# Grzetan/FPV-drone-RL-agent

Hardware: NVIDIA B200
Metric: env-steps/sec (physics+reward+obs), QuadX hover (higher is better)
Workload: dtype f32

## Files before the change

fpv-drone-rl-agent_b200/csrc/qx_kernels.cu:

```cuda
#include <cooperative_groups.h>
#include <cooperative_groups/reduce.h>
#include <cuda_bf16.h>
#include <cuda_runtime.h>

#include <atomic>
#include <cmath>
#include <cstddef>
#include <cstdio>
#include <cstdlib>
#include <cstring>
#include <type_traits>
#include <new>

#include "../../include/quadx_b200.h"
#include "qx_internal.h"
#include "qx_model.cuh"

namespace qx {

#ifndef QX_BLOCK
#define QX_BLOCK 128
#endif
#ifndef QX_MIN_BLOCKS
#define QX_MIN_BLOCKS 4
#endif
#ifndef QX_PAIR_UNROLL
#define QX_PAIR_UNROLL 1
#endif
constexpr int kBlock = QX_BLOCK;

struct Stats {
  double sum_ret;
  unsigned long long sum_len;
  unsigned long long n_done;
  unsigned long long n_nonfinite;
};

struct ResetQueue {
  unsigned int count;
  unsigned int ticket;
  unsigned int tasks_done, next_reset, exit_ticket, published;
  unsigned int pad[2];
  unsigned int idx[1];
};

struct StepArgs {
  float4* state;
  const float* actions;
  void* obs;
  float* reward;
  uint8_t* terminated;
  uint8_t* truncated;
  float* terminal_obs;
  const uint8_t* mask;
  Stats* stats;
  ResetQueue* queue;
  int64_t n;
  int64_t env_begin, env_count;
  int64_t obs_stride;
  int32_t k;
  int32_t obs_bf16;
  int32_t stream_stores;
  int32_t merged;
  uint32_t drainers;
  int32_t paired_reset;
};

template <int DIM>
__device__ __forceinline__ void write_obs(const float (&o)[DIM], void* base, int64_t row, int64_t stride, bool bf16, bool cs = false) {
  static_assert(DIM % 4 == 0, "obs rows are written as 16-byte / 8-byte vectors");
  if (bf16) {
    __nv_bfloat16* p = reinterpret_cast<__nv_bfloat16*>(base) + row * stride;
    if ((stride & 3) == 0) {
#pragma unroll
      for (int j = 0; j < DIM; j += 4) {
        __nv_bfloat162 a = __floats2bfloat162_rn(o[j], o[j + 1]), b = __floats2bfloat162_rn(o[j + 2], o[j + 3]);
        uint2 v;
        v.x = *reinterpret_cast<uint32_t*>(&a);
        v.y = *reinterpret_cast<uint32_t*>(&b);
        if (cs) __stcs(reinterpret_cast<uint2*>(p + j), v);
        else *reinterpret_cast<uint2*>(p + j) = v;
      }
    } else {
#pragma unroll
      for (int j = 0; j < DIM; ++j) p[j] = __float2bfloat16_rn(o[j]);
    }
  } else {
    float* p = reinterpret_cast<float*>(base) + row * stride;
    if ((stride & 3) == 0) {
#pragma unroll
      for (int j = 0; j < DIM; j += 4) {
        if (cs) __stcs(reinterpret_cast<float4*>(p + j), make_float4(o[j], o[j + 1], o[j + 2], o[j + 3]));
        else *reinterpret_cast<float4*>(p + j) = make_float4(o[j], o[j + 1], o[j + 2], o[j + 3]);
      }
    } else {
#pragma unroll
      for (int j = 0; j < DIM; ++j) p[j] = o[j];
    }
  }
}

enum { MODE_STEP_INLINE = 0, MODE_STEP_DEFER = 1, MODE_RESET_MASK = 2, MODE_RESET_QUEUE = 3 };

template <int MODE, int TASK, bool CASC, bool NC = true>
__device__ __forceinline__ void run_env(const DevConfig& c, const StepArgs& a, int64_t i);

constexpr int kResetQueueBlocks = 148 * 4;

__device__ __forceinline__ void publish_queue_length(ResetQueue* q) {
  __syncthreads();
  if (threadIdx.x == 0) {
    if (atomicAdd(&q->tasks_done, 1u) == gridDim.x - 1) {
      q->published = atomicAdd(&q->count, 0u);
      q->tasks_done = 0u;
    }
  }
}

template <int MODE, int TASK, bool CASC = false, bool REF = false>
__global__ void __launch_bounds__(kBlock, QX_MIN_BLOCKS) quadx_step_kernel(const __grid_constant__ DevConfig cparam, const __grid_constant__ StepArgs a) {
  if (MODE == MODE_STEP_INLINE) {
    asm volatile("griddepcontrol.wait;" ::: "memory");
    asm volatile("griddepcontrol.launch_dependents;");
  }
  DevConfig cref = cparam;
  if (REF) apply_ref_constants(cref);
  const DevConfig& c = REF ? cref : cparam;
  if (MODE == MODE_RESET_QUEUE) {
    const unsigned int cnt = *reinterpret_cast<volatile unsigned int*>(&a.queue->count);
    __syncthreads();
    if (threadIdx.x == 0) {
      __threadfence();
      if (atomicAdd(&a.queue->ticket, 1u) == gridDim.x - 1) { a.queue->count = 0u; a.queue->ticket = 0u; }
    }
    for (unsigned int t = blockIdx.x * kBlock + threadIdx.x; t < cnt; t += gridDim.x * kBlock)
      run_env<MODE, TASK, CASC>(c, a, (int64_t)a.queue->idx[t]);
  } else if (MODE == MODE_STEP_DEFER) {
    const int64_t i = a.env_begin + (int64_t)blockIdx.x * kBlock + threadIdx.x;
    if (i < a.env_begin + a.env_count) run_env<MODE, TASK, CASC>(c, a, i);
    publish_queue_length(a.queue);
  } else {
    const int64_t i = a.env_begin + (int64_t)blockIdx.x * kBlock + threadIdx.x;
    if (i >= a.env_begin + a.env_count) return;
    if (MODE == MODE_RESET_MASK && a.mask && !a.mask[i]) return;
    run_env<MODE, TASK, CASC>(c, a, i);
  }
}

__device__ __forceinline__ void respawn_cascade(Env& e, const DevConfig& c, float seul[3], float sp[4]) {
#pragma unroll
  for (int k = 0; k < 18; ++k) e.cp[k] = 0.f;
  quat_to_euler(e.sqx, e.sqy, e.sqz, e.sqw, seul[0], seul[1], seul[2]);
  sp[0] = sp[1] = sp[2] = sp[3] = 0.f;
  if (c.flight_mode == 2 || c.flight_mode == 3 || c.flight_mode == 4) sp[3] = e.spz;
  if (c.flight_mode == 7) { sp[0] = e.spx; sp[1] = e.spy; sp[2] = seul[2]; sp[3] = e.spz; }
}

template <int TASK> struct ObsDim { static constexpr int value = TASK == QX_TASK_HOVER ? QX_OBS_DIM_HOVER : QX_OBS_DIM_YAW; };
struct ObsAux { float er, ep, ey, cx, cy, area, ratio; bool vis; };

template <int TASK, bool RASTER_OK = true>
__device__ __forceinline__ void build_obs(Env& e, const DevConfig& c, const float act[4], const int phase, const bool live,
                                          float (&obs)[ObsDim<TASK>::value], ObsAux& x) {
  float er, ep, ey;
  if (phase == 0 && !live) {
    er = e.peul[0]; ep = e.peul[1]; ey = e.peul[2];
  } else {
    quat_to_euler(e.sqx, e.sqy, e.sqz, e.sqw, er, ep, ey);
  }
  if (phase == 1) { e.peul[0] = er; e.peul[1] = ep; e.peul[2] = ey; }
  const float two_pi = 6.28318530718f, pi = 3.14159265359f;
  float d0 = er - e.peul[0] + pi, d1 = ep - e.peul[1] + pi, d2 = ey - e.peul[2] + pi;
  d0 = d0 - two_pi * floorf(d0 * (1.f / two_pi)) - pi;
  d1 = d1 - two_pi * floorf(d1 * (1.f / two_pi)) - pi;
  d2 = d2 - two_pi * floorf(d2 * (1.f / two_pi)) - pi;
  bool vis;
  float cx, cy, area = 0.f, ratio = 0.f;
  if (TASK == QX_TASK_HOVER) {
    if (RASTER_OK && c.vision_mode == 1) vision_raster(e.px, e.py, e.pz, e.qx, e.qy, e.qz, e.qw, c.raster, vis, cx, cy, area, ratio);
    else vision(e, c, vis, cx, cy, area, ratio);
    obs[0] = d0 * c.inv_agent_dt; obs[1] = d1 * c.inv_agent_dt; obs[2] = d2 * c.inv_agent_dt;
    euler_to_quat(er, ep, ey, obs[3], obs[4], obs[5], obs[6]);
    obs[7] = cx; obs[8] = cy; obs[9] = e.pcx; obs[10] = e.pcy;
    obs[11] = area; obs[12] = e.parea; obs[13] = vis ? 1.f : 0.f; obs[14] = ratio; obs[15] = e.pratio;
    obs[16] = act[0]; obs[17] = act[1]; obs[18] = act[2]; obs[19] = act[3];
    e.pcx = cx; e.pcy = cy; e.parea = area; e.pratio = ratio;
  } else {
    vision_point(e, c, vis, cx, cy);
    const float k = c.inv_agent_dt * (1.f / 30.f);
    obs[0] = er * (1.f / pi); obs[1] = ep * (1.f / pi); obs[2] = ey * (1.f / pi);
    obs[3] = cx; obs[4] = cy;
    obs[5] = clampf(d0 * k, -1.f, 1.f); obs[6] = clampf(d1 * k, -1.f, 1.f); obs[7] = clampf(d2 * k, -1.f, 1.f);
    obs[8] = e.pa[0]; obs[9] = e.pa[1]; obs[10] = e.pa[2]; obs[11] = e.pa[3];
    e.pcx = cx; e.pcy = cy;
  }
  x.er = er; x.ep = ep; x.ey = ey; x.cx = cx; x.cy = cy; x.area = area; x.ratio = ratio; x.vis = vis;
}

template <int TASK, bool CASC>
__device__ __forceinline__ bool reward_and_flags(Env& e, const DevConfig& c, const StepArgs& a, const int64_t row, const float act[4],
                                                 const bool live, float (&obs)[ObsDim<TASK>::value], const ObsAux& x) {
  constexpr int OBS_DIM = ObsDim<TASK>::value;
  if (TASK == QX_TASK_YAW) {
    uint32_t fl = e.flags;
    if (e.step_count >= c.max_steps) fl |= F_TRUNC;
    if (e.spx * e.spx + e.spy * e.spy + e.spz * e.spz > c.dome2) fl |= F_OOB | F_TERM;
    const float reward = (x.vis ? 1.f - fabsf(x.cx) : -1.f) - 0.05f * fabsf(e.pa[3] - e.pa[2]);
    e.flags = fl;
    e.peul[0] = x.er; e.peul[1] = x.ep; e.peul[2] = x.ey;
    e.step_count += 1;
    e.rng_ctr += 1u;
    e.ep_ret += reward;
    a.reward[row] = reward;
    a.terminated[row] = (fl & F_TERM) ? 1 : 0;
    a.truncated[row] = (fl & F_TRUNC) ? 1 : 0;
    return c.auto_reset && (fl & (F_TERM | F_TRUNC));
  }
  float reward = -0.1f;
  uint32_t fl = e.flags;
  if (e.step_count > c.max_steps) fl |= F_TRUNC;
  if (live) {
    fl &= ~(F_LOWZ);
    if (e.spx * e.spx + e.spy * e.spy + e.spz * e.spz > c.dome2) fl |= F_OOB;
    if (e.spz < c.floor_thr) fl |= F_LOWZ;
  }
  bool bad = false;
  if (live && !(fabsf(e.px) + fabsf(e.py) + fabsf(e.pz) + fabsf(e.vx) + fabsf(e.vy) + fabsf(e.vz) + fabsf(e.wx) + fabsf(e.wy) + fabsf(e.wz) +
                fabsf(e.qw) < 3.0e38f)) {
    fl |= F_OOB;
    bad = true;
    atomicAdd(&a.stats->n_nonfinite, 1ull);
    e.px = e.py = 0.f; e.pz = c.floor_z; e.vx = e.vy = e.vz = 0.f; e.wx = e.wy = e.wz = 0.f; e.qx = e.qy = e.qz = 0.f; e.qw = 1.f;
#pragma unroll
    for (int m = 0; m < 4; ++m) e.thr[m] = 0.f;
#pragma unroll
    for (int ax = 0; ax < 3; ++ax) { e.pi[ax] = e.pe[ax] = e.swb[ax] = e.svb[ax] = 0.f; }
    if (CASC) {
#pragma unroll
      for (int k = 0; k < 18; ++k) e.cp[k] = 0.f;
      e.spx = e.spy = 0.f; e.spz = c.floor_z;
    }
  }
  if (fl & F_OOB) { reward = -100.f; fl |= F_TERM; }
  if (e.step_count > c.floor_grace && !c.render && (fl & F_LOWZ)) {
    reward = -100.f; fl |= F_TERM | F_ONFLOOR;
  }
  const float target_reward =
      x.vis ? -(fsqrt(x.cx * x.cx + x.cy * x.cy) + fabsf(x.area - c.target_area) + fabsf(x.ratio - c.target_ratio)) : -2.0f;
  reward -= 0.01f * e.swb[2] * e.swb[2];
  reward += target_reward - fsqrt(x.er * x.er + x.ep * x.ep);
  const float a0 = act[0] - e.pa[0], a1 = act[1] - e.pa[1], a2 = act[2] - e.pa[2], a3 = act[3] - e.pa[3];
  reward -= 0.2f * fsqrt(a0 * a0 + a1 * a1 + a2 * a2 + a3 * a3);
  reward += 1.0f;
  if (bad) {
    reward = -100.f;
#pragma unroll
    for (int j = 0; j < OBS_DIM; ++j) obs[j] = 0.f;
  }
  e.flags = fl;
  e.peul[0] = x.er; e.peul[1] = x.ep; e.peul[2] = x.ey;
  e.step_count += 1;
  e.pa[0] = act[0]; e.pa[1] = act[1]; e.pa[2] = act[2]; e.pa[3] = act[3];
  e.rng_ctr += 1u;
  e.ep_ret += reward;
  const bool term = fl & F_TERM, trunc = fl & F_TRUNC;
  if (a.stream_stores) {
    __stcs(a.reward + row, reward);
    __stcs(a.terminated + row, (uint8_t)(term ? 1 : 0));
    __stcs(a.truncated + row, (uint8_t)(trunc ? 1 : 0));
  } else {
    a.reward[row] = reward;
    a.terminated[row] = term ? 1 : 0;
    a.truncated[row] = trunc ? 1 : 0;
  }
  return c.auto_reset && (term || trunc);
}

template <bool DEFER, int OBS_DIM>
__device__ __forceinline__ void episode_end(const Env& e, const StepArgs& a, const int64_t i, const float (&obs)[OBS_DIM]) {
  namespace cg = cooperative_groups;
  const auto g = cg::coalesced_threads();
  const double sr = cg::reduce(g, (double)e.ep_ret, cg::plus<double>());
  const unsigned long long sl = cg::reduce(g, (unsigned long long)e.step_count, cg::plus<unsigned long long>());
  unsigned int base = 0;
  if (g.thread_rank() == 0) {
    atomicAdd(&a.stats->sum_ret, sr);
    atomicAdd(&a.stats->sum_len, sl);
// ... 199 lines not shown
  sp[3] = vfma(L::make(av0.w, av1.w), c.thrust_scale, c.thrust_bias);
  sp[3] = L::make(__saturatef(half_of<0>(sp[3])), __saturatef(half_of<1>(sp[3])));
  const uint32_t k0a = c.seed_lo ^ (c.env_lo + (uint32_t)i0), k0b = c.seed_lo ^ (c.env_lo + (uint32_t)i1);
  const uint32_t k1a = c.seed_hi ^ (c.env_hi + (uint32_t)(((uint64_t)c.env_lo + (uint64_t)i0) >> 32));
  const uint32_t k1b = c.seed_hi ^ (c.env_hi + (uint32_t)(((uint64_t)c.env_lo + (uint64_t)i1) >> 32));
  const int nsub = c.n_sub_step;
#pragma unroll 1
  for (int j = 0; j < nsub; j += 2) {
    V apwm[4];
    control_update<V>(p, c, sp, apwm);
    V nz[4] = {splat<V>(0.f), splat<V>(0.f), splat<V>(0.f), splat<V>(0.f)};
    uint4 ba = make_uint4(0u, 0u, 0u, 0u), bb = ba;
    if (c.noise) {
      ba = env_philox(make_uint4((uint32_t)j >> 1, STREAM_STEP, e0.rng_ctr, 0u), k0a, k1a);
      if (kLanes == 2) bb = env_philox(make_uint4((uint32_t)j >> 1, STREAM_STEP, e1.rng_ctr, 0u), k0b, k1b);
      if constexpr (kLanes == 2) normal4_scaled<V>(make_uint2(ba.x, bb.x), make_uint2(ba.y, bb.y), c.noise_k, nz);
      else normal4_scaled<V>(ba.x, ba.y, c.noise_k, nz);
    }
    physics_substep<V>(p, c, apwm, nz, false);
    if (c.noise) {
      if constexpr (kLanes == 2) normal4_scaled<V>(make_uint2(ba.z, bb.z), make_uint2(ba.w, bb.w), c.noise_k, nz);
      else normal4_scaled<V>(ba.z, ba.w, c.noise_k, nz);
    }
    physics_substep<V>(p, c, apwm, nz, j + 2 == nsub);
  }
  unpack_lane<0>(e0, p);
  if (kLanes == 2) unpack_lane<1>(e1, p);
}

#ifndef QX_SWP
#define QX_SWP 0
#endif
#ifndef QX_DIAG
#define QX_DIAG 0
#endif
#ifndef QX_RESET_SWP
#define QX_RESET_SWP 0
#endif
template <bool FLOOR = true, int SWP = QX_SWP>
QX_DI float substeps_s(const DevConfig& c, Env& e0, const f2 spxy, const float spz, const float thrust, const int nsub, const uint32_t stream, const int64_t i0) {
  CoreS p;
  pack_core_s(p, e0);
  float minz = __int_as_float(0x7f800000);
  const uint32_t k0 = c.seed_lo ^ (c.env_lo + (uint32_t)i0);
  const uint32_t k1 = c.seed_hi ^ (c.env_hi + (uint32_t)(((uint64_t)c.env_lo + (uint64_t)i0) >> 32));
  if constexpr (SWP == 0) {
#pragma unroll 1
  for (int j = 0; j < nsub; j += 2) {
    f2 apwm[2];
    control_update_s(p, c, spxy, spz, thrust, apwm);
    f2 nz[2] = {f2{0.f, 0.f}, f2{0.f, 0.f}};
    uint4 b = make_uint4(0u, 0u, 0u, 0u);
    if (c.noise) {
#if QX_DIAG == 2
      b = make_uint4(k0 + j, k1 ^ j, e0.rng_ctr * 0x9E3779B9u + j, k0 * 0x85EBCA6Bu + j);
#else
      b = env_philox(make_uint4((uint32_t)j >> 1, stream, e0.rng_ctr, 0u), k0, k1);
#endif
#if QX_DIAG == 1
      nz[0] = vmul(f2{__uint_as_float(0x3f800000u | (b.x >> 9)) - 1.5f, __uint_as_float(0x3f800000u | (b.x << 14 >> 9)) - 1.5f}, 0.02f);
      nz[1] = vmul(f2{__uint_as_float(0x3f800000u | (b.y >> 9)) - 1.5f, __uint_as_float(0x3f800000u | (b.y << 14 >> 9)) - 1.5f}, 0.02f);
#else
      normal4_scaled_s(b.x, b.y, c.noise_k, nz);
#endif
    }
    physics_substep_s<FLOOR>(p, c, apwm, nz, false, minz);
#if QX_DIAG == 1
    if (c.noise) {
      nz[0] = vmul(f2{__uint_as_float(0x3f800000u | (b.z >> 9)) - 1.5f, __uint_as_float(0x3f800000u | (b.z << 14 >> 9)) - 1.5f}, 0.02f);
      nz[1] = vmul(f2{__uint_as_float(0x3f800000u | (b.w >> 9)) - 1.5f, __uint_as_float(0x3f800000u | (b.w << 14 >> 9)) - 1.5f}, 0.02f);
    }
#else
    if (c.noise) normal4_scaled_s(b.z, b.w, c.noise_k, nz);
#endif
    physics_substep_s<FLOOR>(p, c, apwm, nz, j + 2 == nsub, minz);
  }
  } else if constexpr (SWP == 1) {
  uint4 b = make_uint4(0u, 0u, 0u, 0u);
  if (c.noise) b = env_philox(make_uint4(0u, stream, e0.rng_ctr, 0u), k0, k1);
#pragma unroll 1
  for (int j = 0; j < nsub; j += 2) {
    const uint4 bc = b;
    if (c.noise && j + 2 < nsub) b = env_philox(make_uint4(((uint32_t)j >> 1) + 1u, stream, e0.rng_ctr, 0u), k0, k1);
    f2 apwm[2];
    control_update_s(p, c, spxy, spz, thrust, apwm);
    f2 nz[2] = {f2{0.f, 0.f}, f2{0.f, 0.f}};
    if (c.noise) normal4_scaled_s(bc.x, bc.y, c.noise_k, nz);
    physics_substep_s<FLOOR>(p, c, apwm, nz, false, minz);
    if (c.noise) normal4_scaled_s(bc.z, bc.w, c.noise_k, nz);
    physics_substep_s<FLOOR>(p, c, apwm, nz, j + 2 == nsub, minz);
  }
  } else {
  f2 na[2] = {f2{0.f, 0.f}, f2{0.f, 0.f}}, nb[2] = {f2{0.f, 0.f}, f2{0.f, 0.f}};
  if (c.noise) {
    const uint4 b = env_philox(make_uint4(0u, stream, e0.rng_ctr, 0u), k0, k1);
    normal4_scaled_s(b.x, b.y, c.noise_k, na);
    normal4_scaled_s(b.z, b.w, c.noise_k, nb);
  }
#pragma unroll 1
  for (int j = 0; j < nsub; j += 2) {
    const f2 ca[2] = {na[0], na[1]}, cb[2] = {nb[0], nb[1]};
    if (c.noise && j + 2 < nsub) {
      const uint4 b = env_philox(make_uint4(((uint32_t)j >> 1) + 1u, stream, e0.rng_ctr, 0u), k0, k1);
      normal4_scaled_s(b.x, b.y, c.noise_k, na);
      normal4_scaled_s(b.z, b.w, c.noise_k, nb);
    }
    f2 apwm[2];
    control_update_s(p, c, spxy, spz, thrust, apwm);
    physics_substep_s<FLOOR>(p, c, apwm, ca, false, minz);
    physics_substep_s<FLOOR>(p, c, apwm, cb, j + 2 == nsub, minz);
  }
  }
  unpack_core_s(e0, p);
  return minz;
}
template <>
QX_DI void hot_substeps<S1>(const DevConfig& c, Env& e0, Env&, const float4 av0, const float4, const int64_t i0, const int64_t) {
  const f2 spxy = vmul(f2{av0.x, av0.y}, cpair(c.act_scale[0], c.act_scale[1]));
  const float spz = __fmul_rn(av0.z, c.act_scale[2]);
  const float thrust = __saturatef(fmaf(av0.w, c.thrust_scale, c.thrust_bias));
  substeps_s(c, e0, spxy, spz, thrust, c.n_sub_step, STREAM_STEP, i0);
}
#ifndef QX_SPEC_FLOOR
#define QX_SPEC_FLOOR 1
#endif
#ifndef QX_PREFETCH_TAIL
#define QX_PREFETCH_TAIL 1
#endif
QX_DI void hot_substeps_spec(const DevConfig& c, Env& e0, const StepArgs& a, const float4 av0, const int64_t i0) {
  const f2 spxy = vmul(f2{av0.x, av0.y}, cpair(c.act_scale[0], c.act_scale[1]));
  const float spz = __fmul_rn(av0.z, c.act_scale[2]);
  const float thrust = __saturatef(fmaf(av0.w, c.thrust_scale, c.thrust_bias));
  const float T = __fmul_rn((float)c.n_sub_step, c.h);
  const float reach = fmaf(fminf(e0.vz, 0.f), T, e0.pz) - __fmul_rn(__fmul_rn(c.g, T), T);
  const bool risky = e0.contact || !(reach > c.floor_z);
  const bool slow = __any_sync(__activemask(), risky);
  float minz = __int_as_float(0x7f800000);
  if (!slow) minz = substeps_s<false>(c, e0, spxy, spz, thrust, c.n_sub_step, STREAM_STEP, i0);
  const bool redo = minz < c.floor_z;
  if (slow || redo) {
    if (redo) load_env_loop(e0, a.state, a.n, i0);
    substeps_s<true>(c, e0, spxy, spz, thrust, c.n_sub_step, STREAM_STEP, i0);
  }
}

template <bool NC>
QX_DI void hot_reset_env(const DevConfig& c, const StepArgs& a, const int64_t i) {
  constexpr int OBS_DIM = QX_OBS_DIM_HOVER;
  Env e;
  load_env<NC>(e, a.state, a.n, i);
  const uint32_t k0 = c.seed_lo ^ (c.env_lo + (uint32_t)i);
  const uint32_t k1 = c.seed_hi ^ (c.env_hi + (uint32_t)(((uint64_t)c.env_lo + (uint64_t)i) >> 32));
  respawn(e, c, k0, k1);
  substeps_s<true, QX_RESET_SWP>(c, e, f2{0.f, 0.f}, 0.f, 0.f, c.n_sub_reset, STREAM_RESET, i);
  const float act[4] = {0.f, 0.f, 0.f, 0.f};
  float obs[OBS_DIM];
  ObsAux x;
  build_obs<QX_TASK_HOVER, false>(e, c, act, 1, true, obs, x);
  if (a.obs) write_obs(obs, a.obs, i, a.obs_stride, a.obs_bf16 != 0);
  store_env(e, a.state, a.n, i);
}
template <bool REF>
__device__ __noinline__ void hot_reset_requeue(const DevConfig& cparam, const StepArgs& a, const int64_t i) {
  DevConfig cref = cparam;
  if (REF) apply_ref_constants(cref);
  const DevConfig& c = REF ? cref : cparam;
  hot_reset_env<false>(c, a, i);
}

template <bool REF, class V>
QX_DI void hot_task(const DevConfig& c, const DevConfig& cparam, const StepArgs& a, const int64_t i0, const int64_t i1, const bool has1) {
  constexpr int kLanes = Lane<V>::N;
  Env e0, e1;
  const float4 av0 = __ldg(reinterpret_cast<const float4*>(a.actions) + i0);
  const float4 av1 = kLanes == 2 ? __ldg(reinterpret_cast<const float4*>(a.actions) + i1) : av0;
  load_env_loop(e0, a.state, a.n, i0);
  if (kLanes == 2) load_env_loop(e1, a.state, a.n, i1);
  if ((e0.flags | (kLanes == 2 ? e1.flags : 0u)) & (F_TERM | F_TRUNC)) {
    run_env_cold<REF>(cparam, a, i0);
    if (has1) run_env_cold<REF>(cparam, a, i1);
    return;
  }
#if QX_PREFETCH_TAIL
#pragma unroll
  for (int p = kLoopPlanes; p < 11; ++p) asm volatile("prefetch.global.L2 [%0];" ::"l"(a.state + (int64_t)p * a.n + i0));
#endif
  if constexpr (QX_SPEC_FLOOR && std::is_same<V, S1>::value) hot_substeps_spec(c, e0, a, av0, i0);
  else hot_substeps<V>(c, e0, e1, av0, av1, i0, i1);
  hot_epilogue<REF>(e0, c, a, i0, av0);
  if (has1) hot_epilogue<REF>(e1, c, a, i1, av1);
}

QX_DI unsigned int ld_acquire_u32(const unsigned int* p) {
  unsigned int v;
  asm volatile("ld.acquire.gpu.global.u32 %0, [%1];" : "=r"(v) : "l"(p) : "memory");
  return v;
}

template <bool REF, int SHAPE, class V, bool MERGED>
__global__ void __launch_bounds__(HotShape<SHAPE>::kBlock, HotShape<SHAPE>::kMinBlocks) quadx_step_hot_kernel(const __grid_constant__ DevConfig cparam,
                                                                                                                 const __grid_constant__ StepArgs a) {
  constexpr int kB = HotShape<SHAPE>::kBlock, kLanes = Lane<V>::N, kWarps = kB / 32, kTask = 32 * kLanes;
  if constexpr (!MERGED) {
    asm volatile("griddepcontrol.wait;" ::: "memory");
    asm volatile("griddepcontrol.launch_dependents;");
  }
  DevConfig cref = cparam;
  if (REF) apply_ref_constants(cref);
  const DevConfig& c = REF ? cref : cparam;
  const int64_t end = a.env_begin + a.env_count;
  const int64_t i0 = a.env_begin + ((int64_t)blockIdx.x * kWarps + (threadIdx.x >> 5)) * kTask + (threadIdx.x & 31u);
  if (i0 < end) {
    const bool has1 = kLanes == 2 && i0 + 32 < end;
    hot_task<REF, V>(c, cparam, a, i0, has1 ? i0 + 32 : i0, has1);
  }
  if constexpr (!MERGED) {
    if (a.queue) publish_queue_length(a.queue);
  }
  if constexpr (MERGED) {
    ResetQueue* const q = a.queue;
    __shared__ unsigned int s_ticket;
    __syncthreads();
    if (threadIdx.x == 0) s_ticket = atomicAdd(&q->tasks_done, 1u);
    __syncthreads();
    if (s_ticket + a.drainers < gridDim.x) return;
    if (threadIdx.x == 0) {
      unsigned int ns = 64u;
      while (ld_acquire_u32(&q->tasks_done) < gridDim.x) { __nanosleep(ns); if (ns < 512u) ns += ns; }
    }
    __syncthreads();
    const unsigned int cnt = ld_acquire_u32(&q->count);
#pragma unroll 1
    while (cnt != 0u) {
      unsigned int r = 0u;
      if ((threadIdx.x & 31u) == 0u) r = atomicAdd(&q->next_reset, 32u);
      r = __shfl_sync(0xffffffffu, r, 0);
      if (r >= cnt) break;
      if (r + (threadIdx.x & 31u) < cnt) {
        const int64_t ie = (int64_t)__ldcg(&q->idx[r + (threadIdx.x & 31u)]);
        if (a.paired_reset) hot_reset_requeue<REF>(cparam, a, ie);
        else run_env_requeue<REF>(cparam, a, ie);
      }
      __syncwarp();
    }
    __syncthreads();
    if (threadIdx.x == 0) {
      const unsigned int n_drain = a.drainers < gridDim.x ? a.drainers : gridDim.x;
      if (atomicAdd(&q->exit_ticket, 1u) == n_drain - 1u) {
        q->published = cnt; q->count = 0u; q->tasks_done = 0u; q->next_reset = 0u; q->exit_ticket = 0u;
      }
    }
  }
}

template <bool REF>
__global__ void __launch_bounds__(128, 4) quadx_reset_hot_kernel(const __grid_constant__ DevConfig cparam, const __grid_constant__ StepArgs a) {
  DevConfig cref = cparam;
  if (REF) apply_ref_constants(cref);
  const DevConfig& c = REF ? cref : cparam;
  asm volatile("griddepcontrol.wait;" ::: "memory");
  asm volatile("griddepcontrol.launch_dependents;");
  const unsigned int cnt = *reinterpret_cast<volatile unsigned int*>(&a.queue->count);
  __syncthreads();
  if (threadIdx.x == 0) {
    __threadfence();
    if (atomicAdd(&a.queue->ticket, 1u) == gridDim.x - 1) { a.queue->count = 0u; a.queue->ticket = 0u; }
  }
  for (unsigned int t = blockIdx.x * 128 + threadIdx.x; t < cnt; t += gridDim.x * 128) hot_reset_env<true>(c, a, (int64_t)a.queue->idx[t]);
}

__global__ void clock_probe_kernel(unsigned long long* out) {
  unsigned long long ns;
  asm volatile("mov.u64 %0, %%globaltimer;" : "=l"(ns));
  out[0] = (unsigned long long)clock64();
  out[1] = ns;
}

}

struct QxHandle {
  QxConfig cfg;
  qx::DevConfig dev;
  int64_t n;
  int device;
  int planes;
  bool ref_constants;
  bool hot_ok;
  int hot_mode;
  int paired_reset;
  int hot_lanes;
  int hot_shape;
  int stream_stores;
  int merged;
  int sm_count;
  int pdl;
  int host_chunks;
  int host_one_d2h;
  int hot_grid;
  float4* state;
  qx::Stats* stats;
  qx::ResetQueue* queue;
  float* raster;
  cudaStream_t stream, h2d_stream, d2h_stream, d2h2_stream;
  cudaEvent_t ev_h2d[16], ev_k[16], ev_d2h;
  float* h_act; float* d_act;
  float* h_obs; float* d_obs;
  float* h_rew; float* d_rew;
  uint8_t* h_flags; uint8_t* d_flags;
  float* h_tobs; float* d_tobs;
  bool staging;
};

static thread_local char g_err[512] = "";
static std::atomic<int64_t> g_launches{0};

int qx_fail(int code, const char* fmt, const char* detail) {
  snprintf(g_err, sizeof(g_err), fmt, detail);
  return code;
}
static int fail(int code, const char* fmt, const char* detail = "") { return qx_fail(code, fmt, detail); }
#define QX_CUDA(call)                                                             \
  do {                                                                            \
    cudaError_t _e = (call);                                                      \
    if (_e != cudaSuccess) return fail(QX_ECUDA, #call ": %s", cudaGetErrorString(_e)); \
  } while (0)

extern "C" const char* qx_last_error(void) { return g_err; }
extern "C" int32_t qx_version(void) { return QX_VERSION; }
extern "C" int64_t qx_launch_count(void) { return g_launches.load(); }
extern "C" int64_t qx_sizeof_config(void) { return (int64_t)sizeof(QxConfig); }

extern "C" int qx_default_config(int32_t task, QxConfig* c) {
  if (!c || (task != QX_TASK_HOVER && task != QX_TASK_YAW)) return fail(QX_EINVAL, "qx_default_config: bad arguments");
  memset(c, 0, sizeof(*c));
  c->task = task;
  c->mass = 0.1f;
  c->inertia[0] = 3e-5f; c->inertia[1] = 3e-5f; c->inertia[2] = 5e-5f;
  const float mx[4] = {0.028f, -0.028f, 0.028f, -0.028f}, my[4] = {-0.028f, 0.028f, 0.028f, -0.028f};
  const float ts[4] = {-1.f, -1.f, 1.f, 1.f};
  const float map[16] = {-1, -1, -1, 1, 1, 1, -1, 1, 1, -1, 1, 1, -1, 1, 1, 1};
  memcpy(c->motor_x, mx, sizeof(mx)); memcpy(c->motor_y, my, sizeof(my));
  memcpy(c->torque_sign, ts, sizeof(ts)); memcpy(c->motor_map, map, sizeof(map));
  c->total_thrust = 4.0f; c->thrust_coef = 3.16e-10f; c->torque_coef = 7.94e-12f; c->noise_ratio = 0.02f; c->tau = 0.01f;
  c->drag_coef_xyz = 1.5f; c->drag_area_xyz = 3.0e-4f; c->drag_coef_pqr = 1.0e-4f; c->air_density = 1.225f;
  const float kp[3] = {2.0e-2f, 2.0e-2f, 4.0e-2f}, ki[3] = {2.5e-7f, 2.5e-7f, 1.35e-4f}, kd[3] = {5.0e-5f, 5.0e-5f, 0.f};
  for (int a = 0; a < 3; ++a) { c->rate_kp[a] = kp[a]; c->rate_ki[a] = ki[a]; c->rate_kd[a] = kd[a]; c->rate_lim[a] = 1.0f; }
  c->pwm_idle = 0.05f; c->physics_hz = 240.f; c->control_hz = 120.f; c->gravity = 9.81f;
  c->state_stale = 1; c->gyro = 1; c->max_coord_vel = 100.f; c->floor_z = 0.01f;
  c->cam_tilt_up_deg = 25.f; c->cam_fov_deg = 90.f; c->cam_res = 128.f; c->cam_near = 0.1f; c->vis_margin_px = 0.5f;
  const float panel[12] = {4.98f, -1, 5, 4.98f, 1, 5, 4.98f, 1, 7, 4.98f, -1, 7};
  memcpy(c->panel, panel, sizeof(panel));
  for (int k = 0; k < 4; ++k) { c->panel_back[3 * k] = panel[3 * k] + 0.04f; c->panel_back[3 * k + 1] = panel[3 * k + 1]; c->panel_back[3 * k + 2] = panel[3 * k + 2]; }
  c->vision_mode = 0;
  c->aviary_steps_per_step = task == QX_TASK_HOVER ? 6 : 1;
  c->max_steps = 400; c->floor_grace_steps = 30; c->reset_idle_steps = task == QX_TASK_HOVER ? 10 : 0;
  c->agent_dt = 0.025f; c->flight_dome_size = 3.0f; c->floor_threshold = 0.1f;
  c->target_area = 0.013f; c->target_ratio = 1.53f;
  c->action_scale[0] = 30.f; c->action_scale[1] = 30.f; c->action_scale[2] = -30.f;
  c->spawn_yaw_noise = task == QX_TASK_YAW ? 3.14159265f : 0.f;
  if (task == QX_TASK_YAW) {
    c->cam_tilt_up_deg = -20.f;
    c->panel[0] = 2.f; c->panel[1] = 0.f; c->panel[2] = 1.f;
    c->agent_dt = 1.0f / 120.f;
  }
  c->render = 0; c->auto_reset = 1; c->noise = 1;
  c->flight_mode = 0; c->thrust_scale = 0.5f; c->thrust_bias = 0.5f;
  const float att[12] = {1, 1, 1, 0, 0, 0, 0, 0, 0, 2, 2, 2};
  const float vel[8] = {0.4f, 0.4f, 0.15f, 0.15f, 0.25f, 0.25f, 0.3f, 0.3f};
  const float pos[8] = {0.5f, 0.5f, 0, 0, 0, 0, 1, 1};
  const float zp[4] = {0.8f, 0, 0, 1.5f}, zv[4] = {1.5f, 0.3f, 0.05f, 1.0f};
  memcpy(c->att_pid, att, sizeof(att)); memcpy(c->vel_pid, vel, sizeof(vel)); memcpy(c->pos_pid, pos, sizeof(pos));
  memcpy(c->zpos_pid, zp, sizeof(zp)); memcpy(c->zvel_pid, zv, sizeof(zv));
  return QX_OK;
}

static int derive(const QxConfig& s, uint64_t seed, uint64_t env_id0, qx::DevConfig* d) {
  memset(d, 0, sizeof(*d));
  if (s.task != QX_TASK_HOVER && s.task != QX_TASK_YAW) return fail(QX_EINVAL, "qx_create: unknown task");
  if (!(s.physics_hz > 0) || !(s.control_hz > 0) || s.control_hz > s.physics_hz) return fail(QX_EINVAL, "qx_create: bad rates");
  if (s.flight_mode < -1 || s.flight_mode > 7) return fail(QX_EINVAL, "qx_create: flight_mode outside PyFlyt's -1..7");
  if (s.flight_mode != 0 && s.task != QX_TASK_HOVER) return fail(QX_EINVAL, "qx_create: flight modes other than 0 apply to the hover task");
  if (s.vision_mode != 0 && s.vision_mode != 1) return fail(QX_EINVAL, "qx_create: vision_mode is 0 (analytic) or 1 (raster)");
  const int per = (int)(s.physics_hz / s.control_hz);
  d->task = s.task;
  d->ctrl_every = per;
  d->n_sub_step = s.aviary_steps_per_step * per;
  d->n_sub_reset = s.reset_idle_steps * per;
  d->max_steps = s.max_steps; d->floor_grace = s.floor_grace_steps; d->render = s.render; d->auto_reset = s.auto_reset;
  d->noise = (s.noise && s.noise_ratio != 0.f) ? 1 : 0;
  d->state_stale = s.state_stale; d->gyro = s.gyro;
  d->obs_dim = s.task == QX_TASK_HOVER ? QX_OBS_DIM_HOVER : QX_OBS_DIM_YAW;
  d->act_dim = s.task == QX_TASK_HOVER ? QX_ACT_DIM_HOVER : QX_ACT_DIM_YAW;
  const double h = 1.0 / s.physics_hz, T = 1.0 / s.control_hz;
  d->h = (float)h; d->lag_alpha = (float)(h / s.tau); d->one_m_alpha = (float)(1.0 - h / s.tau); d->noise_ratio = s.noise_ratio;
  d->noise_k = (float)(-2.0 * M_LN2 * (double)s.noise_ratio * (double)s.noise_ratio);
  d->thrust_k = (float)(s.total_thrust / 4.0); d->pwm_idle = s.pwm_idle;
  const double max_rpm2 = s.total_thrust / (4.0 * s.thrust_coef);
  for (int m = 0; m < 4; ++m) {
    d->torque_k[m] = (float)(s.torque_sign[m] * s.torque_coef * max_rpm2);
    d->mx[m] = s.motor_x[m]; d->my[m] = s.motor_y[m];
  }
  memcpy(d->map, s.motor_map, sizeof(d->map));
  d->drag_c = (float)(0.5 * s.air_density * s.drag_coef_xyz * s.drag_area_xyz); d->drag_pqr = s.drag_coef_pqr;
  for (int a = 0; a < 3; ++a) {
    d->kp[a] = s.rate_kp[a]; d->kiT[a] = (float)(s.rate_ki[a] * T); d->kd_T[a] = (float)(s.rate_kd[a] / T); d->lim[a] = s.rate_lim[a];
    d->I[a] = s.inertia[a]; d->invI[a] = (float)(1.0 / s.inertia[a]);
    d->cam_off[a] = s.cam_offset[a]; d->act_scale[a] = s.action_scale[a];
    d->start_pos[a] = s.start_pos[a]; d->start_rpy[a] = s.start_rpy[a];
  }
  d->inv_mass = (float)(1.0 / s.mass); d->g = s.gravity; d->vmax = s.max_coord_vel; d->floor_z = s.floor_z;
  for (int a = 0; a < 3; ++a) {
    d->hI[a] = (float)(h / s.inertia[a]);
    d->gk[a] = s.gyro ? (float)(-(h / s.inertia[a]) * ((double)s.inertia[(a + 2) % 3] - (double)s.inertia[(a + 1) % 3])) : 0.f;
  }
  d->hm = (float)(h / s.mass); d->hg = (float)(h * s.gravity); d->hh = (float)(0.5 * h); d->hh2 = (float)(0.25 * h * h);
  d->kq1 = (float)(-0.5 * h / 6.0); d->kq2 = (float)(0.5 * h / 120.0);
  d->ndrag_c = -(float)(0.5 * s.air_density * s.drag_coef_xyz * s.drag_area_xyz); d->ndrag_pqr = -s.drag_coef_pqr;
  const double tilt = s.cam_tilt_up_deg * M_PI / 180.0;
  d->cam_sd = (float)sin(tilt); d->cam_cd = (float)cos(tilt);
  d->inv_tan = (float)(1.0 / tan(0.5 * s.cam_fov_deg * M_PI / 180.0));
// ... 115 lines not shown
  return QX_OK;
}

struct DeviceGuard {
  int prev = 0;
  explicit DeviceGuard(int d) { cudaGetDevice(&prev); cudaSetDevice(d); }
  ~DeviceGuard() { cudaSetDevice(prev); }
};

extern "C" int qx_nonfinite_count(QxHandle* h, int64_t* count) {
  if (!h || !count) return fail(QX_EINVAL, "qx_nonfinite_count: bad arguments");
  DeviceGuard g(h->device);
  qx::Stats s;
  QX_CUDA(cudaMemcpy(&s, h->stats, sizeof(s), cudaMemcpyDeviceToHost));
  *count = (int64_t)s.n_nonfinite;
  return QX_OK;
}

extern "C" int64_t qx_num_envs(const QxHandle* h) { return h ? h->n : 0; }
extern "C" int32_t qx_obs_dim(const QxHandle* h) { return h ? h->dev.obs_dim : 0; }
extern "C" int32_t qx_act_dim(const QxHandle* h) { return h ? h->dev.act_dim : 0; }
extern "C" void* qx_state_ptr(QxHandle* h) { return h ? h->state : nullptr; }
extern "C" int32_t qx_state_words(const QxHandle* h) { return h ? 4 * h->planes : 0; }
static bool matches_ref_constants(const qx::DevConfig& d) {
  qx::DevConfig lit = d;
  qx::apply_ref_constants(lit);
  return QX_HAVE_REF_CONSTANTS && d.task == QX_TASK_HOVER && d.flight_mode == 0 && memcmp(&lit, &d, sizeof(lit)) == 0;
}
extern "C" int32_t qx_uses_reference_constants(const QxHandle* h) { return h && h->ref_constants ? 1 : 0; }
extern "C" int32_t qx_config_matches_reference_constants(const QxConfig* cfg) {
  qx::DevConfig d;
  if (!cfg || derive(*cfg, 0, 0, &d) != QX_OK) return -1;
  return matches_ref_constants(d) ? 1 : 0;
}
extern "C" int64_t qx_debug_dev_config(const QxConfig* cfg, uint64_t seed, uint64_t env_id0, void* out, int64_t cap) {
  qx::DevConfig d;
  if (!cfg || derive(*cfg, seed, env_id0, &d) != QX_OK) return -1;
  if (out && cap >= (int64_t)sizeof(d)) memcpy(out, &d, sizeof(d));
  return (int64_t)sizeof(d);
}

template <int TASK, bool CASC, bool REF>
static void launch_task(QxHandle* h, int mode, const qx::StepArgs& a, cudaStream_t s) {
  const unsigned grid = (unsigned)((a.env_count + qx::kBlock - 1) / qx::kBlock);
  switch (mode) {
    case qx::MODE_STEP_INLINE:
      if (h->pdl) {
        cudaLaunchConfig_t lc{};
        lc.gridDim = dim3(grid); lc.blockDim = dim3(qx::kBlock); lc.dynamicSmemBytes = 0; lc.stream = s;
        cudaLaunchAttribute at{};
        at.id = cudaLaunchAttributeProgrammaticStreamSerialization;
        at.val.programmaticStreamSerializationAllowed = 1;
        lc.attrs = &at; lc.numAttrs = 1;
        cudaLaunchKernelEx(&lc, qx::quadx_step_kernel<qx::MODE_STEP_INLINE, TASK, CASC, REF>, h->dev, a);
      } else {
        qx::quadx_step_kernel<qx::MODE_STEP_INLINE, TASK, CASC, REF><<<grid, qx::kBlock, 0, s>>>(h->dev, a);
      }
      break;
    case qx::MODE_STEP_DEFER: qx::quadx_step_kernel<qx::MODE_STEP_DEFER, TASK, CASC, REF><<<grid, qx::kBlock, 0, s>>>(h->dev, a); break;
    case qx::MODE_RESET_MASK: qx::quadx_step_kernel<qx::MODE_RESET_MASK, TASK, CASC, REF><<<grid, qx::kBlock, 0, s>>>(h->dev, a); break;
    default: {
      const unsigned g = grid < (unsigned)qx::kResetQueueBlocks ? grid : (unsigned)qx::kResetQueueBlocks;
      qx::quadx_step_kernel<qx::MODE_RESET_QUEUE, TASK, CASC, REF><<<g, qx::kBlock, 0, s>>>(h->dev, a);
      break;
    }
  }
}

static bool stream_is_capturing(cudaStream_t s) {
  cudaStreamCaptureStatus st = cudaStreamCaptureStatusNone;
  return cudaStreamIsCapturing(s, &st) == cudaSuccess && st != cudaStreamCaptureStatusNone;
}

template <bool REF, int SHAPE, class V>
static cudaError_t launch_hot_kernel(QxHandle* h, const qx::StepArgs& a, cudaStream_t s) {
  constexpr int B = qx::HotShape<SHAPE>::kBlock, per = 32 * qx::Lane<V>::N, warps = B / 32;
  const int64_t n_tasks = (a.env_count + per - 1) / per;
  unsigned grid = (unsigned)((n_tasks + warps - 1) / warps);
  if (a.merged) {
    if (h->hot_grid == 0) {
      int per_sm = 0;
      cudaError_t e = cudaOccupancyMaxActiveBlocksPerMultiprocessor(&per_sm, qx::quadx_step_hot_kernel<REF, SHAPE, V, true>, B, 0);
      if (e != cudaSuccess) return e;
      h->hot_grid = h->sm_count * (per_sm > 0 ? per_sm : 1);
    }
    qx::StepArgs am = a;
    am.drainers = (uint32_t)h->hot_grid;
    qx::quadx_step_hot_kernel<REF, SHAPE, V, true><<<grid, B, 0, s>>>(h->dev, am);
    return cudaSuccess;
  }
  if (h->pdl && !stream_is_capturing(s)) {
    cudaLaunchConfig_t lc{};
    lc.gridDim = dim3(grid); lc.blockDim = dim3(B); lc.dynamicSmemBytes = 0; lc.stream = s;
    cudaLaunchAttribute at{};
    at.id = cudaLaunchAttributeProgrammaticStreamSerialization;
    at.val.programmaticStreamSerializationAllowed = 1;
    lc.attrs = &at; lc.numAttrs = 1;
    return cudaLaunchKernelEx(&lc, qx::quadx_step_hot_kernel<REF, SHAPE, V, false>, h->dev, a);
  }
  qx::quadx_step_hot_kernel<REF, SHAPE, V, false><<<grid, B, 0, s>>>(h->dev, a);
  return cudaSuccess;
}
template <int SHAPE, class V>
static cudaError_t launch_hot_one(QxHandle* h, const qx::StepArgs& a, cudaStream_t s) {
  return h->ref_constants ? launch_hot_kernel<true, SHAPE, V>(h, a, s) : launch_hot_kernel<false, SHAPE, V>(h, a, s);
}
template <class V>
static cudaError_t launch_hot_shape(QxHandle* h, const qx::StepArgs& a, cudaStream_t s) {
  switch (h->hot_shape) {
    case 3: return launch_hot_one<3, V>(h, a, s);
    case 4: return launch_hot_one<4, V>(h, a, s);
    case 5: return launch_hot_one<5, V>(h, a, s);
    default: return launch_hot_one<0, V>(h, a, s);
  }
}
static bool use_merged(const QxHandle* h);
static int launch_hot(QxHandle* h, int mode, qx::StepArgs a, cudaStream_t s) {
  if (a.env_count == 0) { a.env_begin = 0; a.env_count = h->n; }
  a.stream_stores = h->stream_stores;
  a.merged = (mode == qx::MODE_STEP_DEFER && use_merged(h)) ? h->merged : 0;
  a.paired_reset = h->paired_reset;
  if (a.merged) a.queue = h->queue;
  cudaError_t e;
#ifdef QX_EXTRA_SHAPES
  if (h->hot_lanes == 4 && h->hot_shape >= 6) {
    switch (h->hot_shape) {
      case 6: e = launch_hot_one<6, qx::S1>(h, a, s); break;
      case 7: e = launch_hot_one<7, qx::S1>(h, a, s); break;
      case 8: e = launch_hot_one<8, qx::S1>(h, a, s); break;
      default: e = launch_hot_one<9, qx::S1>(h, a, s); break;
    }
  } else
#endif
  if (h->hot_lanes == 2) e = launch_hot_shape<qx::P2<true>>(h, a, s);
  else if (h->hot_lanes == 4) e = launch_hot_shape<qx::S1>(h, a, s);
  else e = launch_hot_shape<float>(h, a, s);
  QX_CUDA(e);
  ++g_launches;
  QX_CUDA(cudaGetLastError());
  return QX_OK;
}
constexpr int64_t kHotMinEnvs = 32768;
static bool use_hot(const QxHandle* h) {
  if (!h->hot_ok || h->hot_mode == 0) return false;
  return h->hot_mode == 1 || h->n >= kHotMinEnvs;
}
static bool use_merged(const QxHandle* h) { return use_hot(h) && h->cfg.auto_reset && h->merged; }

static int launch(QxHandle* h, int mode, qx::StepArgs a, cudaStream_t s) {
  if (a.env_count == 0) { a.env_begin = 0; a.env_count = h->n; }
  if (use_hot(h) && (mode == qx::MODE_STEP_DEFER || (mode == qx::MODE_STEP_INLINE && a.k == 1 && !h->cfg.auto_reset)))
    return launch_hot(h, mode, a, s);
  if (mode == qx::MODE_RESET_QUEUE && use_hot(h) && h->paired_reset) {
    const unsigned blocks = (unsigned)((a.env_count + 127) / 128);
    const unsigned g = blocks < (unsigned)qx::kResetQueueBlocks ? blocks : (unsigned)qx::kResetQueueBlocks;
    if (h->pdl && !stream_is_capturing(s)) {
      cudaLaunchConfig_t lc{};
      lc.gridDim = dim3(g); lc.blockDim = dim3(128); lc.dynamicSmemBytes = 0; lc.stream = s;
      cudaLaunchAttribute at{};
      at.id = cudaLaunchAttributeProgrammaticStreamSerialization;
      at.val.programmaticStreamSerializationAllowed = 1;
      lc.attrs = &at; lc.numAttrs = 1;
      QX_CUDA(h->ref_constants ? cudaLaunchKernelEx(&lc, qx::quadx_reset_hot_kernel<true>, h->dev, a)
                               : cudaLaunchKernelEx(&lc, qx::quadx_reset_hot_kernel<false>, h->dev, a));
    } else if (h->ref_constants) qx::quadx_reset_hot_kernel<true><<<g, 128, 0, s>>>(h->dev, a);
    else qx::quadx_reset_hot_kernel<false><<<g, 128, 0, s>>>(h->dev, a);
    ++g_launches;
    QX_CUDA(cudaGetLastError());
    return QX_OK;
  }
  if (h->dev.task == QX_TASK_YAW) launch_task<QX_TASK_YAW, false, false>(h, mode, a, s);
  else if (h->dev.flight_mode != 0) launch_task<QX_TASK_HOVER, true, false>(h, mode, a, s);
  else if (h->ref_constants) launch_task<QX_TASK_HOVER, false, true>(h, mode, a, s);
  else launch_task<QX_TASK_HOVER, false, false>(h, mode, a, s);
  ++g_launches;
  QX_CUDA(cudaGetLastError());
  return QX_OK;
}

extern "C" int qx_reset(QxHandle* h, const uint8_t* mask_dev, void* obs_dev, int32_t obs_dtype, int64_t obs_stride, void* stream) {
  if (!h) return fail(QX_EINVAL, "qx_reset: null handle");
  if (obs_dev && obs_stride < h->dev.obs_dim) return fail(QX_EINVAL, "qx_reset: obs_stride < obs_dim");
  qx::StepArgs a{};
  a.state = h->state; a.mask = mask_dev; a.obs = obs_dev; a.obs_stride = obs_stride; a.obs_bf16 = obs_dtype == QX_OBS_BF16;
  a.stats = h->stats; a.n = h->n; a.k = 1;
  return launch(h, qx::MODE_RESET_MASK, a, (cudaStream_t)stream);
}

extern "C" int qx_step_k(QxHandle* h, int32_t k, const float* actions_dev, float* obs_dev, float* reward_dev,
                         uint8_t* terminated_dev, uint8_t* truncated_dev, void* stream) {
  if (!h || k <= 0 || !actions_dev || !reward_dev || !terminated_dev || !truncated_dev)
    return fail(QX_EINVAL, "qx_step_k: bad arguments");
  qx::StepArgs a{};
  a.state = h->state; a.actions = actions_dev; a.obs = obs_dev; a.obs_stride = h->dev.obs_dim; a.reward = reward_dev;
  a.terminated = terminated_dev; a.truncated = truncated_dev; a.stats = h->stats; a.n = h->n; a.k = k;
  return launch(h, qx::MODE_STEP_INLINE, a, (cudaStream_t)stream);
}

extern "C" int qx_step_begin(QxHandle* h, const float* actions_dev, void* obs_dev, int32_t obs_dtype, int64_t obs_stride,
                             float* reward_dev, uint8_t* terminated_dev, uint8_t* truncated_dev, float* terminal_obs_dev, void* stream) {
  if (!h || !actions_dev || !reward_dev || !terminated_dev || !truncated_dev) return fail(QX_EINVAL, "qx_step: bad arguments");
  if (obs_dev && obs_stride < h->dev.obs_dim) return fail(QX_EINVAL, "qx_step: obs_stride < obs_dim");
  qx::StepArgs a{};
  a.state = h->state; a.actions = actions_dev; a.obs = obs_dev; a.obs_stride = obs_stride; a.obs_bf16 = obs_dtype == QX_OBS_BF16;
  a.reward = reward_dev; a.terminated = terminated_dev; a.truncated = truncated_dev; a.terminal_obs = terminal_obs_dev;
  a.stats = h->stats; a.n = h->n; a.k = 1;
  if (!h->cfg.auto_reset) return launch(h, qx::MODE_STEP_INLINE, a, (cudaStream_t)stream);
  a.queue = h->queue;
  return launch(h, qx::MODE_STEP_DEFER, a, (cudaStream_t)stream);
}

extern "C" int qx_step_end(QxHandle* h, void* obs_dev, int32_t obs_dtype, int64_t obs_stride, void* stream) {
  if (!h) return fail(QX_EINVAL, "qx_step_end: null handle");
  if (!h->cfg.auto_reset) return QX_OK;
  if (obs_dev && obs_stride < h->dev.obs_dim) return fail(QX_EINVAL, "qx_step_end: obs_stride < obs_dim");
  if (use_merged(h)) return QX_OK;
  qx::StepArgs a{};
  a.state = h->state; a.obs = obs_dev; a.obs_stride = obs_stride; a.obs_bf16 = obs_dtype == QX_OBS_BF16;
  a.stats = h->stats; a.queue = h->queue; a.n = h->n; a.k = 1;
  return launch(h, qx::MODE_RESET_QUEUE, a, (cudaStream_t)stream);
}

constexpr int64_t kInlineResetMaxEnvs = 16384;
extern "C" int qx_step(QxHandle* h, const float* actions_dev, void* obs_dev, int32_t obs_dtype, int64_t obs_stride,
                       float* reward_dev, uint8_t* terminated_dev, uint8_t* truncated_dev, float* terminal_obs_dev, void* stream) {
  if (h && h->cfg.auto_reset && h->n <= kInlineResetMaxEnvs && !(h->hot_mode == 1 && h->hot_ok)) {
    if (!actions_dev || !reward_dev || !terminated_dev || !truncated_dev) return fail(QX_EINVAL, "qx_step: bad arguments");
    if (obs_dev && obs_stride < h->dev.obs_dim) return fail(QX_EINVAL, "qx_step: obs_stride < obs_dim");
    qx::StepArgs a{};
    a.state = h->state; a.actions = actions_dev; a.obs = obs_dev; a.obs_stride = obs_stride; a.obs_bf16 = obs_dtype == QX_OBS_BF16;
    a.reward = reward_dev; a.terminated = terminated_dev; a.truncated = truncated_dev; a.terminal_obs = terminal_obs_dev;
    a.stats = h->stats; a.n = h->n; a.k = 1;
    return launch(h, qx::MODE_STEP_INLINE, a, (cudaStream_t)stream);
  }
  int rc = qx_step_begin(h, actions_dev, obs_dev, obs_dtype, obs_stride, reward_dev, terminated_dev, truncated_dev, terminal_obs_dev, stream);
  if (rc) return rc;
  return qx_step_end(h, obs_dev, obs_dtype, obs_stride, stream);
}

extern "C" int qx_debug_clock_probe(unsigned long long* out_dev, void* stream) {
  if (!out_dev) return fail(QX_EINVAL, "qx_debug_clock_probe: null buffer");
  qx::clock_probe_kernel<<<1, 1, 0, (cudaStream_t)stream>>>(out_dev);
  QX_CUDA(cudaGetLastError());
  return QX_OK;
}

extern "C" int qx_done_queue(QxHandle* h, const uint32_t** count_dev, const uint32_t** idx_dev) {
  if (!h || !count_dev || !idx_dev) return fail(QX_EINVAL, "qx_done_queue: bad arguments");
  *count_dev = &h->queue->published;
  *idx_dev = h->queue->idx;
  return QX_OK;
}

static int ensure_staging(QxHandle* h) {
  if (h->staging) return QX_OK;
  const int64_t n = h->n;
  const int od = h->dev.obs_dim, ad = h->dev.act_dim;
  QX_CUDA(cudaMallocHost(&h->h_act, sizeof(float) * n * ad)); QX_CUDA(cudaMalloc(&h->d_act, sizeof(float) * n * ad));
  QX_CUDA(cudaMallocHost(&h->h_obs, sizeof(float) * n * od)); QX_CUDA(cudaMalloc(&h->d_obs, sizeof(float) * n * od));
  QX_CUDA(cudaMallocHost(&h->h_rew, sizeof(float) * n)); QX_CUDA(cudaMalloc(&h->d_rew, sizeof(float) * n));
  QX_CUDA(cudaMallocHost(&h->h_flags, 3 * n)); QX_CUDA(cudaMalloc(&h->d_flags, 3 * n));
  QX_CUDA(cudaMallocHost(&h->h_tobs, sizeof(float) * n * od)); QX_CUDA(cudaMalloc(&h->d_tobs, sizeof(float) * n * od));
  h->staging = true;
  return QX_OK;
}


extern "C" int qx_reset_host(QxHandle* h, const uint8_t* mask_host, float* obs_host) {
  if (!h) return fail(QX_EINVAL, "qx_reset_host: null handle");
  DeviceGuard g(h->device);
  int rc = ensure_staging(h);
  if (rc) return rc;
  const int64_t n = h->n;
  const int od = h->dev.obs_dim;
  uint8_t* dmask = nullptr;
  if (mask_host) {
    memcpy(h->h_flags + 2 * n, mask_host, n);
    QX_CUDA(cudaMemcpyAsync(h->d_flags + 2 * n, h->h_flags + 2 * n, n, cudaMemcpyHostToDevice, h->stream));
    dmask = h->d_flags + 2 * n;
  }
  rc = qx_reset(h, dmask, h->d_obs, QX_OBS_F32, od, h->stream);
  if (rc) return rc;
  if (obs_host) QX_CUDA(cudaMemcpyAsync(h->h_obs, h->d_obs, sizeof(float) * n * od, cudaMemcpyDeviceToHost, h->stream));
  QX_CUDA(cudaStreamSynchronize(h->stream));
  if (obs_host) {
    if (!mask_host) memcpy(obs_host, h->h_obs, sizeof(float) * n * od);
    else
      for (int64_t i = 0; i < n; ++i)
        if (mask_host[i]) memcpy(obs_host + i * od, h->h_obs + i * od, sizeof(float) * od);
  }
  return QX_OK;
}

static bool is_pinned(const void* p) {
  if (!p) return false;
  cudaPointerAttributes at;
  if (cudaPointerGetAttributes(&at, p) != cudaSuccess) { cudaGetLastError(); return false; }
  return at.type == cudaMemoryTypeHost;
}

static int step_host_impl(QxHandle* h, const float* actions_host, void* obs_host, const int32_t obs_dtype, float* reward_host,
                          uint8_t* terminated_host, uint8_t* truncated_host, float* terminal_obs_host) {
  if (!h || !actions_host) return fail(QX_EINVAL, "qx_step_host: bad arguments");
  if (obs_dtype != QX_OBS_F32 && obs_dtype != QX_OBS_BF16) return fail(QX_EINVAL, "qx_step_host: obs_dtype is QX_OBS_F32 or QX_OBS_BF16");
  const bool bf16 = obs_dtype == QX_OBS_BF16;
  const size_t osz = bf16 ? 2 : 4;
  DeviceGuard g(h->device);
  int rc = ensure_staging(h);
// ... 142 lines not shown
```

Baseline: 7.465 billion.

## Hand off reset count via pending field, add fast reset substep path, resize reset grid

The step kernel's last block now atomically swaps the queue count to zero and stores it in a new pending field. Reset kernels read that field directly instead of running their own ticket atomics and fences. The hot reset runs its substeps on a non-contact fast path when no lane can reach the floor, and re-spawns then redoes the slow path if the floor is crossed. The reset grid is sized to SM count times five blocks with matching launch bounds, which adds register pressure and a warp-divergent redo risk.

```diff
diff --git a/fpv-drone-rl-agent_b200/csrc/qx_kernels.cu b/fpv-drone-rl-agent_b200/csrc/qx_kernels.cu
--- a/fpv-drone-rl-agent_b200/csrc/qx_kernels.cu
+++ b/fpv-drone-rl-agent_b200/csrc/qx_kernels.cu
@@ -38,7 +38,7 @@
 
 struct ResetQueue {
   unsigned int count;
-  unsigned int ticket;
+  unsigned int pending;
   unsigned int tasks_done, next_reset, exit_ticket, published;
   unsigned int pad[2];
   unsigned int idx[1];
@@ -111,7 +111,9 @@
   __syncthreads();
   if (threadIdx.x == 0) {
     if (atomicAdd(&q->tasks_done, 1u) == gridDim.x - 1) {
-      q->published = atomicAdd(&q->count, 0u);
+      const unsigned int cnt = atomicExch(&q->count, 0u);
+      q->published = cnt;
+      q->pending = cnt;
       q->tasks_done = 0u;
     }
   }
@@ -127,12 +129,7 @@
   if (REF) apply_ref_constants(cref);
   const DevConfig& c = REF ? cref : cparam;
   if (MODE == MODE_RESET_QUEUE) {
-    const unsigned int cnt = *reinterpret_cast<volatile unsigned int*>(&a.queue->count);
-    __syncthreads();
-    if (threadIdx.x == 0) {
-      __threadfence();
-      if (atomicAdd(&a.queue->ticket, 1u) == gridDim.x - 1) { a.queue->count = 0u; a.queue->ticket = 0u; }
-    }
+    const unsigned int cnt = a.queue->pending;
     for (unsigned int t = blockIdx.x * kBlock + threadIdx.x; t < cnt; t += gridDim.x * kBlock)
       run_env<MODE, TASK, CASC>(c, a, (int64_t)a.queue->idx[t]);
   } else if (MODE == MODE_STEP_DEFER) {
@@ -638,7 +635,16 @@
   const uint32_t k0 = c.seed_lo ^ (c.env_lo + (uint32_t)i);
   const uint32_t k1 = c.seed_hi ^ (c.env_hi + (uint32_t)(((uint64_t)c.env_lo + (uint64_t)i) >> 32));
   respawn(e, c, k0, k1);
-  substeps_s<true, QX_RESET_SWP>(c, e, f2{0.f, 0.f}, 0.f, 0.f, c.n_sub_reset, STREAM_RESET, i);
+  const float T = __fmul_rn((float)c.n_sub_reset, c.h);
+  const float reach = fmaf(fminf(e.vz, 0.f), T, e.pz) - __fmul_rn(__fmul_rn(c.g, T), T);
+  const bool slow = __any_sync(__activemask(), e.contact || !(reach > c.floor_z));
+  float minz = __int_as_float(0x7f800000);
+  if (!slow) minz = substeps_s<false, QX_RESET_SWP>(c, e, f2{0.f, 0.f}, 0.f, 0.f, c.n_sub_reset, STREAM_RESET, i);
+  const bool redo = minz < c.floor_z;
+  if (slow || redo) {
+    if (redo) respawn(e, c, k0, k1);
+    substeps_s<true, QX_RESET_SWP>(c, e, f2{0.f, 0.f}, 0.f, 0.f, c.n_sub_reset, STREAM_RESET, i);
+  }
   const float act[4] = {0.f, 0.f, 0.f, 0.f};
   float obs[OBS_DIM];
   ObsAux x;
@@ -739,19 +745,15 @@
   }
 }
 
+constexpr int kResetHotBlocksPerSM = 5;
 template <bool REF>
-__global__ void __launch_bounds__(128, 4) quadx_reset_hot_kernel(const __grid_constant__ DevConfig cparam, const __grid_constant__ StepArgs a) {
+__global__ void __launch_bounds__(128, kResetHotBlocksPerSM) quadx_reset_hot_kernel(const __grid_constant__ DevConfig cparam, const __grid_constant__ StepArgs a) {
   DevConfig cref = cparam;
   if (REF) apply_ref_constants(cref);
   const DevConfig& c = REF ? cref : cparam;
   asm volatile("griddepcontrol.wait;" ::: "memory");
   asm volatile("griddepcontrol.launch_dependents;");
-  const unsigned int cnt = *reinterpret_cast<volatile unsigned int*>(&a.queue->count);
-  __syncthreads();
-  if (threadIdx.x == 0) {
-    __threadfence();
-    if (atomicAdd(&a.queue->ticket, 1u) == gridDim.x - 1) { a.queue->count = 0u; a.queue->ticket = 0u; }
-  }
+  const unsigned int cnt = a.queue->pending;
   for (unsigned int t = blockIdx.x * 128 + threadIdx.x; t < cnt; t += gridDim.x * 128) hot_reset_env<true>(c, a, (int64_t)a.queue->idx[t]);
 }
 
@@ -1173,8 +1175,8 @@
   if (use_hot(h) && (mode == qx::MODE_STEP_DEFER || (mode == qx::MODE_STEP_INLINE && a.k == 1 && !h->cfg.auto_reset)))
     return launch_hot(h, mode, a, s);
   if (mode == qx::MODE_RESET_QUEUE && use_hot(h) && h->paired_reset) {
-    const unsigned blocks = (unsigned)((a.env_count + 127) / 128);
-    const unsigned g = blocks < (unsigned)qx::kResetQueueBlocks ? blocks : (unsigned)qx::kResetQueueBlocks;
+    const unsigned blocks = (unsigned)((a.env_count + 127) / 128), wave = (unsigned)(h->sm_count * qx::kResetHotBlocksPerSM);
+    const unsigned g = blocks < wave ? blocks : wave;
     if (h->pdl && !stream_is_capturing(s)) {
       cudaLaunchConfig_t lc{};
       lc.gridDim = dim3(g); lc.blockDim = dim3(128); lc.dynamicSmemBytes = 0; lc.stream = s;
```

After: 7.468 billion, median of 6. Within noise of the previous version (+0.0%).
